# openfheorg/openfhe-development

Hardware: AMD Instinct MI355X
Metric: NTT GB/s vs HBM roofline + CKKS EvalMultKeySwitch/sec, N=2^16 L=30, 1/2/4/8 GPU (higher is better)
Workload: dtype u64; 1 GPU; batched fwd+inv negacyclic NTT, N=2^16, L=30 x 60-bit limbs, 1024 polynomials per GPU (BASELINE configs[1]); global_batch=1024, parallelism=batch-sharded x1, no data-path collective

## Files before the change

openfhe-development_amd/csrc/basis_kernels.h:

```cpp
#ifndef FHE_BASIS_KERNELS_H
#define FHE_BASIS_KERNELS_H
#include <type_traits>

#include "modarith.h"
#include "launch.h"
#include "ntt_kernels.h"
#include "elemwise_kernels.h"
#include "ntt_static.h"

namespace fhe {


struct ConvTables {
    const TwPair* hatInv;
    const uint64_t* hatMod;
    const uint64_t* srcQ;
    const uint64_t* dstQ;
    const uint64_t* dstMu;
    const uint64_t* dstRed;
    const double* srcQInv;
    const uint64_t* alphaMod;
};

struct ConvArgs {
    const uint64_t* in;
    uint64_t* out;
    ConvTables tb;
    uint32_t logN, batch;
    uint32_t nSrc, nDst;
    uint32_t inStride, inFirst, outStride, outFirst;
    uint32_t acc;
    uint32_t last;
    uint32_t nSrcAll;
    const uint64_t* inAll;
    const TwPair* allHatInv;
    const uint64_t* allSrcQ;
    const double* allQInv;
};

template <int NSRC, bool EXACT, int SUM8 = 2, bool CHUNK = false>
FHE_GLOBAL void FHE_LAUNCH_BOUNDS(kThreads) switch_basis_kernel(const ConvArgs g) {
    const uint32_t N     = 1u << g.logN;
    const uint64_t gid   = (uint64_t)FHE_BID * kThreads + FHE_TID;
    if (gid >= ((uint64_t)g.batch << g.logN))
        return;
    const uint32_t b  = (uint32_t)(gid >> g.logN);
    const uint32_t ri = (uint32_t)gid & (N - 1u);
    const uint64_t* in = g.in + (((uint64_t)b * g.inStride + g.inFirst) << g.logN) + ri;
    uint64_t* out      = g.out + (((uint64_t)b * g.outStride + g.outFirst) << g.logN) + ri;

    uint64_t xin[NSRC];
#pragma unroll
    for (int i = 0; i < NSRC; ++i) {
        const uint32_t row = (uint32_t)i < g.nSrc ? (uint32_t)i : g.nSrc - 1u;
        xin[i]             = in[(uint64_t)row << g.logN];
    }
    uint64_t y[NSRC];
    double nu = 0.5;
    const uint64_t* hp = reinterpret_cast<const uint64_t*>(g.tb.hatInv);
#pragma unroll
    for (int i = 0; i < NSRC; ++i) {
        const uint64_t w = FHE_ULOAD64(hp, 2 * i), wp = FHE_ULOAD64(hp, 2 * i + 1), qi = FHE_ULOAD64(g.tb.srcQ, i);
        const double qinv = EXACT ? FHE_ULOADF64(g.tb.srcQInv, i) : 0.0;
        y[i] = 0;
        if (i < (int)g.nSrc) {
            y[i] = mul_shoup(xin[i], w, wp, qi);
            if (EXACT)
                nu += (double)y[i] * qinv;
        }
    }
    if (CHUNK && EXACT && g.last) {
        nu = 0.5;
        const uint64_t* hpa = reinterpret_cast<const uint64_t*>(g.allHatInv);
        const uint64_t* ina = g.inAll + (((uint64_t)b * g.inStride) << g.logN) + ri;
        for (uint32_t i = 0; i < g.nSrcAll; ++i) {
            const uint64_t yi = mul_shoup(ina[(uint64_t)i << g.logN], hpa[2 * i], hpa[2 * i + 1], g.allSrcQ[i]);
            nu += (double)yi * g.allQInv[i];
        }
    }
    const uint32_t alpha = EXACT && (!CHUNK || g.last) ? (uint32_t)nu : 0u;

    for (uint32_t j = 0; j < g.nDst; ++j) {
        uint64_t h[NSRC];
#pragma unroll
        for (int i = 0; i < NSRC; ++i)
            h[i] = FHE_ULOAD64(g.tb.hatMod, (uint64_t)j * NSRC + i);
        const uint64_t p = FHE_ULOAD64(g.tb.dstQ, j);
        const uint64_t mulo = FHE_ULOAD64(g.tb.dstMu, 2 * j), muhi = FHE_ULOAD64(g.tb.dstMu, 2 * j + 1);
        if (SUM8 == 2) {
            const uint32_t k = 64u - (uint32_t)__builtin_clzll(p);
            uint64_t v       = 0;
#pragma unroll
            for (int c0 = 0; c0 < NSRC; c0 += 8) {
                if (c0 && c0 >= (int)g.nSrc)
                    break;
                sum8s s8;
                sum8s_clear(s8);
#pragma unroll
                for (int i = c0; i < c0 + 8 && i < NSRC; ++i) {
                    uint32_t y0, y1, h0, h1;
                    split30(y[i], y0, y1);
                    split30(h[i], h0, h1);
                    sum8s_add(s8, y0, y1, h0, h1);
                }
                const uint64_t rj = sum8s_reduce(s8, p, k, mulo, muhi);
                v                 = c0 ? add_mod(v, rj, p) : rj;
            }
            if (CHUNK && g.acc)
                v = add_mod(v, out[(uint64_t)j << g.logN], p);
            if (EXACT && (!CHUNK || g.last))
                v = sub_mod(v, g.tb.alphaMod[(uint64_t)alpha * g.nDst + j], p);
            out[(uint64_t)j << g.logN] = v;
            continue;
        }
        {
            static_assert(SUM8 == 1 || SUM8 == 2, "SUM8 selects one of the two column-sum forms");
            const uint32_t k = 64u - (uint32_t)__builtin_clzll(p);
            uint64_t v       = 0;
#pragma unroll
            for (int c0 = 0; c0 < NSRC; c0 += 8) {
                if (c0 && c0 >= (int)g.nSrc)
                    break;
                sum8 s8;
                sum8_clear(s8);
#pragma unroll
                for (int i = c0; i < c0 + 8 && i < NSRC; ++i)
                    sum8_add(s8, y[i], h[i]);
                const uint64_t rj = sum8_reduce(s8, p, k, mulo, muhi);
                v                 = c0 ? add_mod(v, rj, p) : rj;
            }
            if (CHUNK && g.acc)
                v = add_mod(v, out[(uint64_t)j << g.logN], p);
            if (EXACT && (!CHUNK || g.last))
                v = sub_mod(v, g.tb.alphaMod[(uint64_t)alpha * g.nDst + j], p);
            out[(uint64_t)j << g.logN] = v;
        }
    }
}

constexpr int kMaxDigits = 8;
struct KsInnerArgs {
    const uint64_t* c;
    const uint64_t* digits[kMaxDigits];
    const uint64_t* keyB;
    const uint64_t* keyA;
    uint64_t* out0;
    uint64_t* out1;
    const LimbConst* lc;
    const uint64_t* mu128;
    const uint64_t* red;
    uint32_t logN, batch, sizeQl, sizeQ, sizeP, numDigits, alpha;
    uint32_t nc[kMaxDigits];
    uint32_t j0, acc;
};
FHE_GLOBAL void FHE_LAUNCH_BOUNDS(kThreads) ks_inner_product_kernel(const KsInnerArgs g) {
    const uint32_t t          = FHE_TID;
    const uint32_t tilesPerRow = (1u << g.logN) >> kTileLog ? ((1u << g.logN) >> kTileLog) : 1u;
    const uint32_t sizeQlP    = g.sizeQl + g.sizeP;
    const uint32_t xcd = FHE_BID & 7u, slot = FHE_BID >> 3;
    const uint32_t b   = slot % g.batch;
    const uint32_t grp = (slot / g.batch) * 8u + xcd;
    const uint32_t tr = grp % tilesPerRow;
    const uint32_t i  = grp / tilesPerRow;
    if (i >= sizeQlP)
        return;
    const uint32_t idx  = i < g.sizeQl ? i : i + (g.sizeQ - g.sizeQl);
    const LimbConst lc  = g.lc[idx];
    const uint64_t mulo = g.mu128[2 * idx], muhi = g.mu128[2 * idx + 1];
    const uint64_t redc = g.red[idx];
    const uint32_t redM = (uint32_t)redc, redR = (uint32_t)(redc >> 32);
    FHE_BOUND_CHECK(redR == 255u || redR >= 3u, "key switch: the quotient estimate on a modulus below 36 bits");
    const uint32_t N    = 1u << g.logN;
    const uint32_t rEnd = ((tr + 1u) << kTileLog) < N ? ((tr + 1u) << kTileLog) : N;
    const uint64_t q = lc.q;
    for (uint32_t r = (tr << kTileLog) + t; r < rEnd; r += kThreads) {
        sum8 s0, s1;
        sum8_clear(s0);
        sum8_clear(s1);
        for (uint32_t j = 0; j < g.numDigits; ++j) {
            const uint32_t start = (g.j0 + j) * g.alpha;
            const uint32_t sz    = sizeQlP - g.nc[j];
            uint64_t d;
            if (i >= start && i < start + sz)
                d = g.c[(((uint64_t)b * g.sizeQl + i) << g.logN) + r];
            else {
                const uint32_t pos = i < start ? i : i - sz;
                d = g.digits[j][(((uint64_t)b * g.nc[j] + pos) << g.logN) + r];
            }
            if (redR != 255u)
                d -= (uint64_t)((uint32_t)(((d >> 32) * redM) >> 32) >> redR) * q;
            else {
                d = csub(d, q << 3);
                d = csub(d, q << 2);
                d = csub(d, q << 1);
            }
            d = csub(d, q);
            FHE_BOUND_CHECK(d < q, "key switch: a digit of q or more enters the 64-bit column sums");
            const uint64_t koff = (((uint64_t)(g.j0 + j) * (g.sizeQ + g.sizeP) + idx) << g.logN) + r;
            sum8_add(s0, d, g.keyB[koff]);
            sum8_add(s1, d, g.keyA[koff]);
        }
        const uint64_t ooff = (((uint64_t)b * sizeQlP + i) << g.logN) + r;
        uint64_t v0 = sum8_reduce(s0, q, lc.msb, mulo, muhi), v1 = sum8_reduce(s1, q, lc.msb, mulo, muhi);
        if (g.acc) {
            v0 = add_mod(v0, g.out0[ooff], q);
            v1 = add_mod(v1, g.out1[ooff], q);
        }
        g.out0[ooff] = v0;
        g.out1[ooff] = v1;
    }
}

constexpr int kMaxMultiKeys = 16;
struct KsInnerMultiArgs {
    const uint64_t* c;
    const uint64_t* digits[kMaxDigits];
    const uint64_t* keyB[kMaxMultiKeys];
    const uint64_t* keyA[kMaxMultiKeys];
    uint64_t* out0[kMaxMultiKeys];
    uint64_t* out1[kMaxMultiKeys];
    const uint64_t* first;
    const TwPair* firstC;
    const LimbConst* lc;
    const uint64_t* mu128;
    const uint64_t* red;
    uint32_t logN, batch, sizeQl, sizeQ, sizeP, numDigits, alpha, nKeys;
    uint32_t nc[kMaxDigits];
};
struct alignas(16) U64x2 {
    uint64_t a, b;
};
template <int CPL>
FHE_HD void ld_cpl(const uint64_t* p, uint64_t (&v)[CPL]) {
    if constexpr (CPL == 2) {
        const U64x2 w = *reinterpret_cast<const U64x2*>(p);
        v[0] = w.a, v[1] = w.b;
    }
    else
        v[0] = p[0];
}
template <int CPL>
FHE_HD void st_cpl(uint64_t* p, const uint64_t (&v)[CPL]) {
    if constexpr (CPL == 2)
        *reinterpret_cast<U64x2*>(p) = U64x2{v[0], v[1]};
    else
        p[0] = v[0];
}
template <int ND, int CPL = 1, bool PF = true>
FHE_GLOBAL void FHE_LAUNCH_BOUNDS(kThreads) ks_inner_multi_kernel(const KsInnerMultiArgs g) {
    const uint32_t t           = FHE_TID;
    const uint32_t tilesPerRow = (1u << g.logN) >> kTileLog ? ((1u << g.logN) >> kTileLog) : 1u;
    const uint32_t sizeQlP     = g.sizeQl + g.sizeP;
    const uint32_t xcd = FHE_BID & 7u, slot = FHE_BID >> 3;
    const uint32_t b   = slot % g.batch;
    const uint32_t grp = (slot / g.batch) * 8u + xcd;
    const uint32_t tr = grp % tilesPerRow;
    const uint32_t i  = grp / tilesPerRow;
    if (i >= sizeQlP)
        return;
    const uint32_t idx  = i < g.sizeQl ? i : i + (g.sizeQ - g.sizeQl);
    const LimbConst lc  = g.lc[idx];
    const uint64_t mulo = g.mu128[2 * idx], muhi = g.mu128[2 * idx + 1];
    const uint64_t redc = g.red[idx];
    const uint32_t redM = (uint32_t)redc, redR = (uint32_t)(redc >> 32);
    FHE_BOUND_CHECK(redR == 255u || redR >= 3u, "key switch: the quotient estimate on a modulus below 36 bits");
    const bool addFirst = g.first != nullptr && i < g.sizeQl;
    TwPair fc{0, 0};
    if (addFirst)
        fc = g.firstC[i];
    const uint32_t N    = 1u << g.logN;
    const uint32_t rEnd = ((tr + 1u) << kTileLog) < N ? ((tr + 1u) << kTileLog) : N;
    const uint64_t q = lc.q;
    const uint64_t ooff0 = ((uint64_t)b * sizeQlP + i) << g.logN;
    const uint64_t* src[ND];
    uint64_t koffJ[ND];
#pragma unroll
    for (int j = 0; j < ND; ++j) {
        const uint32_t jj    = (uint32_t)j < g.numDigits ? (uint32_t)j : g.numDigits - 1u;
        const uint32_t start = jj * g.alpha;
        const uint32_t sz    = sizeQlP - g.nc[jj];
        const bool own       = i >= start && i < start + sz;
        const uint32_t pos   = i < start ? i : i - sz;
        src[j] = own ? g.c + (((uint64_t)b * g.sizeQl + i) << g.logN) : g.digits[jj] + (((uint64_t)b * g.nc[jj] + pos) << g.logN);
        koffJ[j] = ((uint64_t)jj * (g.sizeQ + g.sizeP) + idx) << g.logN;
    }
    const uint64_t* firstRow = addFirst ? g.first + (((uint64_t)b * g.sizeQl + i) << g.logN) : nullptr;
    for (uint32_t r = (tr << kTileLog) + CPL * t; r < rEnd; r += CPL * kThreads) {
        uint64_t d[ND][CPL];
#pragma unroll
        for (int j = 0; j < ND; ++j)
            ld_cpl<CPL>(src[j] + r, d[j]);
        uint64_t fraw[CPL] = {};
        if (addFirst)
            ld_cpl<CPL>(firstRow + r, fraw);
        uint64_t kb[ND][CPL], ka[ND][CPL], nb[ND][CPL], na[ND][CPL];
#pragma unroll
        for (int j = 0; j < ND; ++j) {
            ld_cpl<CPL>(g.keyB[0] + koffJ[j] + r, kb[j]);
            ld_cpl<CPL>(g.keyA[0] + koffJ[j] + r, ka[j]);
        }
// ... 458 lines not shown
```

openfhe-development_amd/csrc/fhe_hip.cpp:

```cpp
#include "../../include/fhe_hip.h"

#include <algorithm>
#include <cmath>
#include <cstdio>
#include <cstdlib>
#include <map>
#include <mutex>
#include <shared_mutex>
#include <string>
#include <type_traits>
#include <vector>

#include "basis_kernels.h"
#include "bfv_kernels.h"
#include "elemwise_kernels.h"
#include "host_math.h"
#include "keygen_kernels.h"
#include "encrypt_kernels.h"
#include "decrypt_kernels.h"
#include "ntt_kernels.h"
#include "ntt_static.h"
#include "ntt_row8.h"
#include "rt.h"
#include "sampler_kernels.h"
// ... 1475 lines not shown
    a.nBlocks = kind == 0 ? (a.total + 255) / 256 : (a.total + 511) / 512;
    return kind == 0   ? blake2_launch<0>(c, a, key, counter0, st)
           : kind == 1 ? blake2_launch<1>(c, a, key, counter0, st)
                       : blake2_launch<2>(c, a, key, counter0, st);
}
extern "C" fhe_status fhe_sample_uniform_blake2(fhe_ctx* c, uint64_t* out, const uint32_t* li, uint32_t nl, uint32_t bt,
                                                const uint32_t key[16], uint64_t counter0, void* st) {
    return blake2_sample(c, out, li, nl, bt, 0, 0.0, key, counter0, st, "fhe_sample_uniform_blake2");
}
extern "C" fhe_status fhe_sample_gaussian_blake2(fhe_ctx* c, uint64_t* out, const uint32_t* li, uint32_t nl, uint32_t bt, double sigma,
                                                 const uint32_t key[16], uint64_t counter0, void* st) {
    return blake2_sample(c, out, li, nl, bt, 1, sigma, key, counter0, st, "fhe_sample_gaussian_blake2");
}
extern "C" fhe_status fhe_sample_ternary_blake2(fhe_ctx* c, uint64_t* out, const uint32_t* li, uint32_t nl, uint32_t bt,
                                                const uint32_t key[16], uint64_t counter0, void* st) {
    return blake2_sample(c, out, li, nl, bt, 2, 0.0, key, counter0, st, "fhe_sample_ternary_blake2");
}

struct fhe_conv {
    fhe_ctx* ctx;
    uint32_t nSrc, nDst;
    std::vector<uint32_t> srcIdx, dstIdx;
    ConvTables tb;
    std::vector<ConvTables> chunks;
    const TwPair* allHatInv  = nullptr;
    const uint64_t* allSrcQ  = nullptr;
    const double* allQInv    = nullptr;
    std::vector<void*> owned;
};

static uint32_t conv_nsrc_pad(uint32_t nSrc) { return nSrc <= 8 ? 8u : nSrc <= 16 ? 16u : 32u; }
static fhe_status conv_from_tables(fhe_ctx* c, const std::vector<uint64_t>& src, const std::vector<uint64_t>& dst,
                                   const uint64_t* hatInvIn, const uint64_t* hatModIn, const uint64_t* alphaIn,
                                   const double* qInvIn, fhe_conv** out) {
    const uint32_t nSrc = (uint32_t)src.size(), nDst = (uint32_t)dst.size();
    if (nSrc < 1 || nSrc > (uint32_t)kMaxLimbs || nDst < 1 || nDst > (uint32_t)kMaxLimbs)
        return fail(FHE_ERR_ARG, "basis conversion: 1..256 source and target limbs");
    fhe_conv* cv = new fhe_conv;
    cv->ctx      = c;
    cv->nSrc     = nSrc;
    cv->nDst     = nDst;
    std::vector<uint64_t> mu(2 * (size_t)nDst), alphaMod((size_t)(nSrc + 1) * nDst, 0), red(4 * (size_t)nDst);
    for (uint32_t j = 0; j < nDst; ++j) {
        host::mu128(dst[j], &mu[2 * j]);
        const uint64_t R = (uint64_t)((((unsigned __int128)1) << 64) % dst[j]);
        red[4 * j]       = dst[j];
        red[4 * j + 1]   = R;
        red[4 * j + 2]   = host::shoup(R, dst[j]);
        red[4 * j + 3]   = (uint64_t)((((unsigned __int128)1) << 64) / dst[j]);
    }
    if (alphaIn)
        for (size_t k = 0; k < alphaMod.size(); ++k)
            alphaMod[k] = alphaIn[k] % dst[k % nDst];
    ConvTables shared{};
    fhe_status s;
    if ((s = dev_copy(&cv->owned, dst.data(), dst.size(), &shared.dstQ)) ||
        (s = dev_copy(&cv->owned, mu.data(), mu.size(), &shared.dstMu)) ||
        (s = dev_copy(&cv->owned, red.data(), red.size(), &shared.dstRed)) ||
        (s = dev_copy(&cv->owned, alphaMod.data(), alphaMod.size(), &shared.alphaMod))) {
        fhe_conv_destroy(cv);
        return s;
    }
    for (uint32_t c0 = 0; c0 < nSrc; c0 += 32u) {
        const uint32_t n   = std::min(32u, nSrc - c0);
        const uint32_t pad = conv_nsrc_pad(n);
        std::vector<TwPair> hatInv(32, TwPair{0, 0});
        std::vector<uint64_t> hatMod((size_t)pad * nDst, 0), srcPad(32, 1);
        std::vector<double> qInv(32, 0.0);
        for (uint32_t i = 0; i < n; ++i) {
            const uint64_t inv = hatInvIn[c0 + i] % src[c0 + i];
            hatInv[i]          = TwPair{inv, host::shoup(inv, src[c0 + i])};
            qInv[i]            = qInvIn ? qInvIn[c0 + i] : 1.0 / static_cast<double>(src[c0 + i]);
            srcPad[i]          = src[c0 + i];
            for (uint32_t j = 0; j < nDst; ++j)
                hatMod[(size_t)j * pad + i] = hatModIn[(size_t)(c0 + i) * nDst + j] % dst[j];
        }
        ConvTables tb = shared;
        if ((s = dev_copy(&cv->owned, hatInv.data(), hatInv.size(), &tb.hatInv)) ||
            (s = dev_copy(&cv->owned, hatMod.data(), hatMod.size(), &tb.hatMod)) ||
            (s = dev_copy(&cv->owned, srcPad.data(), srcPad.size(), &tb.srcQ)) ||
            (s = dev_copy(&cv->owned, qInv.data(), qInv.size(), &tb.srcQInv))) {
            fhe_conv_destroy(cv);
            return s;
        }
        cv->chunks.push_back(tb);
    }
    cv->tb = cv->chunks[0];
    if (nSrc > 32u) {
        std::vector<TwPair> allInv(nSrc);
        std::vector<double> allQInv(nSrc);
        for (uint32_t i = 0; i < nSrc; ++i) {
            const uint64_t inv = hatInvIn[i] % src[i];
            allInv[i]          = TwPair{inv, host::shoup(inv, src[i])};
            allQInv[i]         = qInvIn ? qInvIn[i] : 1.0 / static_cast<double>(src[i]);
        }
        if ((s = dev_copy(&cv->owned, allInv.data(), allInv.size(), &cv->allHatInv)) ||
            (s = dev_copy(&cv->owned, src.data(), src.size(), &cv->allSrcQ)) ||
            (s = dev_copy(&cv->owned, allQInv.data(), allQInv.size(), &cv->allQInv))) {
            fhe_conv_destroy(cv);
            return s;
        }
    }
    *out = cv;
    return FHE_OK;
}
static fhe_status conv_build(fhe_ctx* c, const std::vector<uint64_t>& src, const std::vector<uint64_t>& dst, fhe_conv** out,
                             const uint64_t* srcScale = nullptr, const uint64_t* dstScale = nullptr) {
    const uint32_t nSrc = (uint32_t)src.size(), nDst = (uint32_t)dst.size();
    std::vector<uint64_t> hatInv(nSrc), hatMod((size_t)nSrc * nDst), alphaMod((size_t)(nSrc + 1) * nDst);
    for (uint32_t i = 0; i < nSrc; ++i) {
        const uint64_t hat = host::prod_mod(src, (int)i, src[i]);
        hatInv[i]          = host::invmod(hat, src[i]);
        if (srcScale)
            hatInv[i] = host::mulmod(hatInv[i], srcScale[i] % src[i], src[i]);
        for (uint32_t j = 0; j < nDst; ++j) {
            uint64_t v = host::prod_mod(src, (int)i, dst[j]);
            if (dstScale)
                v = host::mulmod(v, dstScale[j] % dst[j], dst[j]);
            hatMod[(size_t)i * nDst + j] = v;
        }
    }
    for (uint32_t j = 0; j < nDst; ++j) {
        const uint64_t Qmod = host::prod_mod(src, -1, dst[j]);
        for (uint32_t a = 0; a <= nSrc; ++a)
            alphaMod[(size_t)a * nDst + j] = host::mulmod(a % dst[j], Qmod, dst[j]);
    }
    return conv_from_tables(c, src, dst, hatInv.data(), hatMod.data(), alphaMod.data(), nullptr, out);
}

extern "C" fhe_status fhe_conv_create(fhe_ctx* c, const uint32_t* srcIdx, uint32_t nSrc, const uint32_t* dstIdx,
                                      uint32_t nDst, fhe_conv** out) {
    ARG_CHECK(c && srcIdx && dstIdx && out, "fhe_conv_create: null argument");
    ARG_CHECK(nSrc >= 1 && nSrc <= (uint32_t)kMaxLimbs && nDst >= 1 && nDst <= (uint32_t)kMaxLimbs, "fhe_conv_create: bad basis size");
    std::vector<uint64_t> src(nSrc), dst(nDst);
    for (uint32_t i = 0; i < nSrc; ++i) {
        ARG_CHECK(srcIdx[i] < c->L, "fhe_conv_create: source limb exceeds context size");
        src[i] = c->q[srcIdx[i]];
    }
    for (uint32_t j = 0; j < nDst; ++j) {
        ARG_CHECK(dstIdx[j] < c->L, "fhe_conv_create: target limb exceeds context size");
        dst[j] = c->q[dstIdx[j]];
    }
    RT_CHECK(rt::set_device(c->device));
    if (fhe_status s = conv_build(c, src, dst, out))
        return s;
    (*out)->srcIdx.assign(srcIdx, srcIdx + nSrc);
    (*out)->dstIdx.assign(dstIdx, dstIdx + nDst);
    return FHE_OK;
}
extern "C" fhe_status fhe_conv_create_custom(fhe_ctx* c, const uint32_t* srcIdx, uint32_t nSrc, const uint32_t* dstIdx,
                                             uint32_t nDst, const uint64_t* hatInv, const uint64_t* hatMod,
                                             const uint64_t* alphaMod, const double* qInv, fhe_conv** out) {
    ARG_CHECK(c && srcIdx && dstIdx && hatInv && hatMod && out, "fhe_conv_create_custom: null argument");
    ARG_CHECK(nSrc >= 1 && nSrc <= (uint32_t)kMaxLimbs && nDst >= 1 && nDst <= (uint32_t)kMaxLimbs, "fhe_conv_create_custom: bad basis size");
    ARG_CHECK((alphaMod == nullptr) == (qInv == nullptr), "fhe_conv_create_custom: alphaMod and qInv go together");
    std::vector<uint64_t> src(nSrc), dst(nDst);
    for (uint32_t i = 0; i < nSrc; ++i) {
        ARG_CHECK(srcIdx[i] < c->L, "fhe_conv_create_custom: source limb exceeds context size");
        src[i] = c->q[srcIdx[i]];
    }
    for (uint32_t j = 0; j < nDst; ++j) {
        ARG_CHECK(dstIdx[j] < c->L, "fhe_conv_create_custom: target limb exceeds context size");
        dst[j] = c->q[dstIdx[j]];
    }
    RT_CHECK(rt::set_device(c->device));
    if (fhe_status s = conv_from_tables(c, src, dst, hatInv, hatMod, alphaMod, qInv, out))
        return s;
    (*out)->srcIdx.assign(srcIdx, srcIdx + nSrc);
    (*out)->dstIdx.assign(dstIdx, dstIdx + nDst);
    return FHE_OK;
}
extern "C" void fhe_conv_destroy(fhe_conv* cv) {
    if (!cv)
        return;
    for (void* p : cv->owned)
        rt::dfree(p);
    delete cv;
}

template <bool EXACT>
static fhe_status conv_run(fhe_conv* cv, const uint64_t* in, uint32_t inStride, uint32_t inFirst, uint64_t* out,
                           uint32_t outStride, uint32_t outFirst, uint32_t batch, void* st) {
    ARG_CHECK(cv && in && out, "fhe_switch_basis: null argument");
    ARG_CHECK(batch >= 1 && inFirst + cv->nSrc <= inStride && outFirst + cv->nDst <= outStride,
              "fhe_switch_basis: limb window exceeds tower stride");
    RT_CHECK(rt::set_device(cv->ctx->device));
    ConvArgs g{};
    g.in = in, g.out = out, g.tb = cv->tb;
    g.logN = cv->ctx->logN, g.batch = batch, g.nSrc = cv->nSrc, g.nDst = cv->nDst;
    g.inStride = inStride, g.inFirst = inFirst, g.outStride = outStride, g.outFirst = outFirst;
    const uint64_t coeffs = (uint64_t)batch << g.logN;
    const uint32_t grid   = (uint32_t)((coeffs + kThreads - 1) / kThreads);
    static const bool split30 = env_u32("FHE_CONV_SUM8", 2) != 1u;
    if (cv->chunks.size() > 1) {
        g.nSrcAll = cv->nSrc, g.inAll = in + ((size_t)inFirst << g.logN);
        g.allHatInv = cv->allHatInv, g.allSrcQ = cv->allSrcQ, g.allQInv = cv->allQInv;
        for (size_t k = 0; k < cv->chunks.size(); ++k) {
            g.tb      = cv->chunks[k];
            g.nSrc    = std::min(32u, cv->nSrc - 32u * (uint32_t)k);
            g.inFirst = inFirst + 32u * (uint32_t)k;
            g.acc     = k > 0;
            g.last    = k + 1 == cv->chunks.size();
            const uint32_t pad = conv_nsrc_pad(g.nSrc);
            if (pad == 8)
                FHE_LAUNCH((switch_basis_kernel<8, EXACT, 2, true>), grid, st, g);
            else if (pad == 16)
                FHE_LAUNCH((switch_basis_kernel<16, EXACT, 2, true>), grid, st, g);
            else
                FHE_LAUNCH((switch_basis_kernel<32, EXACT, 2, true>), grid, st, g);
            LAUNCH_CHECK();
        }
        return FHE_OK;
    }
    const uint32_t pad = conv_nsrc_pad(cv->nSrc);
    if (pad == 8 && split30)
        FHE_LAUNCH((switch_basis_kernel<8, EXACT, 2>), grid, st, g);
    else if (pad == 8)
        FHE_LAUNCH((switch_basis_kernel<8, EXACT, 1>), grid, st, g);
    else if (pad == 16 && split30)
        FHE_LAUNCH((switch_basis_kernel<16, EXACT, 2>), grid, st, g);
    else if (pad == 16)
        FHE_LAUNCH((switch_basis_kernel<16, EXACT, 1>), grid, st, g);
    else if (split30)
        FHE_LAUNCH((switch_basis_kernel<32, EXACT, 2>), grid, st, g);
    else
        FHE_LAUNCH((switch_basis_kernel<32, EXACT, 1>), grid, st, g);
    LAUNCH_CHECK();
    return FHE_OK;
}
extern "C" fhe_status fhe_approx_switch_basis(fhe_conv* cv, const uint64_t* in, uint32_t is, uint32_t ifst,
                                              uint64_t* out, uint32_t os, uint32_t ofst, uint32_t b, void* st) {
    return conv_run<false>(cv, in, is, ifst, out, os, ofst, b, st);
}
extern "C" fhe_status fhe_switch_basis_exact(fhe_conv* cv, const uint64_t* in, uint32_t is, uint32_t ifst,
                                             uint64_t* out, uint32_t os, uint32_t ofst, uint32_t b, void* st) {
    return conv_run<true>(cv, in, is, ifst, out, os, ofst, b, st);
}

extern "C" size_t fhe_expand_crt_basis_workspace_bytes(const fhe_conv* cv, uint32_t batch) {
    return cv ? (((size_t)batch * cv->nSrc) << cv->ctx->logN) * 8 : 0;
}
static fhe_status expand_run(fhe_conv* cv, const uint64_t* x, int inEval, uint64_t* out, int resultEval, int reverseOrder,
                             uint32_t batch, void* ws, size_t wsBytes, void* st, bool exact) {
    ARG_CHECK(cv && x && out && batch >= 1, "fhe_expand_crt_basis: bad argument");
    ARG_CHECK(!cv->srcIdx.empty(), "fhe_expand_crt_basis: the plan must come from fhe_conv_create[_custom]");
    fhe_ctx* c = cv->ctx;
    RT_CHECK(rt::set_device(c->device));
    const uint32_t nQ = cv->nSrc, nP = cv->nDst, tot = nQ + nP;
    const uint32_t qFirst = reverseOrder ? nP : 0, pFirst = reverseOrder ? 0 : nQ;
    const size_t rowB = (size_t)8 << c->logN;
    const uint64_t* coef = x;
    if (inEval) {
        ARG_CHECK(ws && wsBytes >= fhe_expand_crt_basis_workspace_bytes(cv, batch), "fhe_expand_crt_basis: workspace too small");
        if (fhe_status s = ntt_run(c, true, x, (uint64_t*)ws, cv->srcIdx.data(), nQ, batch, st))
            return s;
        coef = (const uint64_t*)ws;
    }
    if (fhe_status s = exact ? conv_run<true>(cv, coef, nQ, 0, out, tot, pFirst, batch, st)
                             : conv_run<false>(cv, coef, nQ, 0, out, tot, pFirst, batch, st))
        return s;
    const uint64_t* qsrc = (resultEval && inEval) ? x : coef;
    uint64_t* qdst       = out + ((size_t)qFirst << c->logN);
    RT_CHECK(rt::d2d_2d(qdst, tot * rowB, qsrc, nQ * rowB, nQ * rowB, batch, (rt::stream_t)st));
    if (resultEval) {
        NttOpts rows;
        rows.src.stride = rows.dst.stride = tot;
        rows.src.first = rows.dst.first = qFirst;
        if (!inEval)
            if (fhe_status s = ntt_run(c, false, out, out, cv->srcIdx.data(), nQ, batch, st, rows))
                return s;
        rows.src.first = rows.dst.first = pFirst;
        return ntt_run(c, false, out, out, cv->dstIdx.data(), nP, batch, st, rows);
    }
    return FHE_OK;
}
extern "C" fhe_status fhe_expand_crt_basis(fhe_conv* cv, const uint64_t* x, int inEval, uint64_t* out, int resultEval,
                                           int reverseOrder, uint32_t batch, void* ws, size_t wsBytes, void* st) {
    return expand_run(cv, x, inEval, out, resultEval, reverseOrder, batch, ws, wsBytes, st, true);
}
// ... 2784 lines not shown
    behz_moduli(h, q, bsk);
    fhe_status s;
    if ((s = behz_pairs(h, mtildeQHatInvModq, q.data(), h->numQ, &h->tb.mtQHatInv)) ||
        (s = behz_matrix(h, QHatModbsk, h->numQ, h->numBsk, bsk.data(), &h->tb.QHatModbsk)) ||
        (s = behz_pairs(h, QModbsk, bsk.data(), h->numBsk, &h->tb.QModbsk)) ||
        (s = behz_pairs(h, mtildeInvModbsk, bsk.data(), h->numBsk, &h->tb.mtInvModbsk)))
        return s;
    std::vector<uint64_t> mt(h->tb.W, 0);
    std::copy(QHatModmtilde, QHatModmtilde + h->numQ, mt.begin());
    uint64_t* d = nullptr;
    if ((s = dev_copy(&h->owned, mt.data(), mt.size(), &d)))
        return s;
    h->tb.QHatModmt    = d;
    h->tb.negQInvModmt = negQInvModmtilde;
    return FHE_OK;
}
extern "C" fhe_status fhe_behz_override_floorq(fhe_behz* h, const uint64_t* tQHatInvModq, const uint64_t* QHatModbsk,
                                               const uint64_t* qInvModbsk, const uint64_t* tQInvModbsk) {
    ARG_CHECK(h && tQHatInvModq && QHatModbsk && qInvModbsk && tQInvModbsk, "fhe_behz_override_floorq: null argument");
    RT_CHECK(rt::set_device(h->ctx->device));
    std::vector<uint64_t> q, bsk;
    behz_moduli(h, q, bsk);
    fhe_status s;
    if ((s = behz_pairs(h, tQHatInvModq, q.data(), h->numQ, &h->tb.tQHatInv)) ||
        (s = behz_matrix(h, QHatModbsk, h->numQ, h->numBsk, bsk.data(), &h->tb.QHatModbsk)) ||
        (s = behz_matrix(h, qInvModbsk, h->numQ, h->numBsk, bsk.data(), &h->tb.qInvModbsk)) ||
        (s = behz_pairs(h, tQInvModbsk, bsk.data(), h->numBsk, &h->tb.tQInvModbsk)))
        return s;
    return FHE_OK;
}
extern "C" fhe_status fhe_behz_override_conv_sk(fhe_behz* h, const uint64_t* BHatInvModb, const uint64_t* BHatModmsk, uint64_t BInvModmsk,
                                                const uint64_t* BHatModq, const uint64_t* BModq) {
    ARG_CHECK(h && BHatInvModb && BHatModmsk && BHatModq && BModq, "fhe_behz_override_conv_sk: null argument");
    RT_CHECK(rt::set_device(h->ctx->device));
    std::vector<uint64_t> q, bsk;
    behz_moduli(h, q, bsk);
    const uint32_t numB = h->numQ;
    const uint64_t msk  = bsk[numB];
    fhe_status s;
    if ((s = behz_pairs(h, BHatInvModb, bsk.data(), numB, &h->tb.BHatInv)) ||
        (s = behz_matrix(h, BHatModq, numB, h->numQ, q.data(), &h->tb.BHatModq)) || (s = behz_pairs(h, BModq, q.data(), h->numQ, &h->tb.BModq)))
        return s;
    std::vector<uint64_t> bm(h->tb.W, 0);
    for (uint32_t i = 0; i < numB; ++i)
        bm[i] = BHatModmsk[i] % msk;
    uint64_t* d = nullptr;
    if ((s = dev_copy(&h->owned, bm.data(), bm.size(), &d)))
        return s;
    h->tb.BHatModmsk = d;
    h->tb.BInvModmsk = TwPair{BInvModmsk % msk, host::shoup(BInvModmsk % msk, msk)};
    return FHE_OK;
}
static bool behz_split30() {
    static const bool on = env_u32("FHE_CONV_SUM8", 2) != 1u;
    return on;
}
static uint32_t coeff_grid(const fhe_ctx* c, uint32_t batch) {
    return (uint32_t)((((uint64_t)batch << c->logN) + kThreads - 1) / kThreads);
}
extern "C" size_t fhe_behz_workspace_bytes(const fhe_behz* h, uint32_t batch) {
    return h ? ((size_t)batch * h->numQ << h->ctx->logN) * 8 : 0;
}
extern "C" fhe_status fhe_behz_q_to_bsk(fhe_behz* h, uint64_t* x, int evalFormat, uint32_t batch, void* ws, size_t wsBytes,
                                        void* st) {
    ARG_CHECK(h && x && batch >= 1, "fhe_behz_q_to_bsk: bad argument");
    fhe_ctx* c = h->ctx;
    RT_CHECK(rt::set_device(c->device));
    const uint32_t tot = h->numQ + h->numBsk;
    BehzArgs g;
    g.tb = h->tb, g.logN = c->logN, g.batch = batch;
    g.outBsk = TowerView{x, tot, h->numQ};
    g.inBsk = g.outBsk, g.outQ = TowerView{x, tot, 0};
    if (evalFormat) {
        ARG_CHECK(ws && wsBytes >= fhe_behz_workspace_bytes(h, batch), "fhe_behz_q_to_bsk: workspace too small");
        uint64_t* coef = (uint64_t*)ws;
        NttOpts rows;
        rows.src.stride = tot, rows.src.first = 0;
        if (fhe_status s = ntt_run(c, true, x, coef, h->qIdx.data(), h->numQ, batch, st, rows))
            return s;
        g.inQ = TowerView{coef, h->numQ, 0};
        if (h->tb.W > (uint32_t)kMaxBfvLimbs)
            FHE_LAUNCH(behz_q_to_bsk_wide_kernel, coeff_grid(c, batch), st, g);
        else if (behz_split30())
            FHE_LAUNCH((behz_q_to_bsk_kernel<true>), coeff_grid(c, batch), st, g);
        else
            FHE_LAUNCH((behz_q_to_bsk_kernel<false>), coeff_grid(c, batch), st, g);
        LAUNCH_CHECK();
        rows.dst.stride = tot, rows.src.first = rows.dst.first = h->numQ;
        return ntt_run(c, false, x, x, h->bskIdx.data(), h->numBsk, batch, st, rows);
    }
    g.inQ = TowerView{x, tot, 0};
    if (h->tb.W > (uint32_t)kMaxBfvLimbs)
        FHE_LAUNCH(behz_q_to_bsk_wide_kernel, coeff_grid(c, batch), st, g);
    else if (behz_split30())
        FHE_LAUNCH((behz_q_to_bsk_kernel<true>), coeff_grid(c, batch), st, g);
    else
        FHE_LAUNCH((behz_q_to_bsk_kernel<false>), coeff_grid(c, batch), st, g);
    LAUNCH_CHECK();
    return fhe_ntt_fwd(c, x, h->allIdx.data(), tot, batch, st);
}
extern "C" fhe_status fhe_behz_floorq(fhe_behz* h, uint64_t* x, uint32_t batch, void* st) {
    ARG_CHECK(h && x && batch >= 1, "fhe_behz_floorq: bad argument");
    RT_CHECK(rt::set_device(h->ctx->device));
    const uint32_t tot = h->numQ + h->numBsk;
    BehzArgs g;
    g.tb = h->tb, g.logN = h->ctx->logN, g.batch = batch;
    g.inQ = g.outQ = TowerView{x, tot, 0};
// ... 1127 lines not shown
```

openfhe-development_amd/csrc/modarith.h:

```cpp
#ifndef FHE_MODARITH_H
#define FHE_MODARITH_H
#include <stdint.h>

#if defined(__HIPCC__) || defined(__HIP_DEVICE_COMPILE__)
#include <hip/hip_runtime.h>
#define FHE_HD __host__ __device__ __forceinline__
#else
#define FHE_HD inline
#endif

namespace fhe {

FHE_HD uint64_t mulhi64(uint64_t a, uint64_t b) {
#if defined(__HIP_DEVICE_COMPILE__)
    return __umul64hi(a, b);
#else
    return (uint64_t)(((unsigned __int128)a * b) >> 64);
#endif
}

FHE_HD uint64_t csub(uint64_t x, uint64_t m) {
    return x >= m ? x - m : x;
}

// ... 108 lines not shown
    mac192_add(m, a, b);
}
#endif
struct u128w;
FHE_HD void mac192_fold(const mac192& m, uint64_t& lo, uint64_t& hi) {
    const uint64_t c1lo = m.c1 << 32, c1hi = (m.c1 >> 32) + ((uint64_t)m.k1 << 32);
    lo = m.c0 + c1lo;
    hi = m.c2 + c1hi + (uint64_t)m.k0 + (lo < c1lo);
}

struct sum8 {
    uint64_t c0, c1, c2;
    uint32_t k0;
};
FHE_HD void sum8_clear(sum8& s) {
    s.c0 = s.c1 = s.c2 = 0;
    s.k0 = 0;
}
FHE_HD void sum8_add(sum8& s, uint64_t x, uint64_t y) {
    const uint32_t xl = (uint32_t)x, xh = (uint32_t)(x >> 32), yl = (uint32_t)y, yh = (uint32_t)(y >> 32);
    const uint64_t lo = (uint64_t)xl * yl + s.c0;
    s.k0 += lo < s.c0;
    s.c0 = lo;
    s.c1 += (uint64_t)xl * yh;
    s.c1 += (uint64_t)xh * yl;
    s.c2 += (uint64_t)xh * yh;
}
FHE_HD uint64_t sum8_reduce(const sum8& s, uint64_t q, uint32_t k, uint64_t mu_lo, uint64_t mu_hi) {
    const uint64_t m = s.c1 << 32, lo = s.c0 + m;
    const uint64_t hi = s.c2 + (s.c1 >> 32) + s.k0 + (lo < m);
    const uint32_t sh = 65u - k;
    const uint64_t mu = (mu_lo >> sh) | (mu_hi << (64u - sh));
    const uint64_t sv = (lo >> (k - 1u)) | (hi << sh);
    uint64_t r        = lo - mulhi64(sv, mu) * q;
    r -= r >= q ? q : 0;
    r -= r >= q ? q : 0;
    return r;
}

struct sum8s {
    uint64_t c0, c1, c2;
};
FHE_HD void sum8s_clear(sum8s& s) { s.c0 = s.c1 = s.c2 = 0; }
FHE_HD void split30(uint64_t x, uint32_t& x0, uint32_t& x1) {
    x0 = (uint32_t)x & 0x3fffffffu;
    x1 = (uint32_t)(x >> 30);
}
FHE_HD void sum8s_add(sum8s& s, uint32_t x0, uint32_t x1, uint32_t y0, uint32_t y1) {
    s.c0 += (uint64_t)x0 * y0;
    s.c1 += (uint64_t)x0 * y1;
    s.c1 += (uint64_t)x1 * y0;
    s.c2 += (uint64_t)x1 * y1;
}
FHE_HD uint64_t sum8s_reduce(const sum8s& s, uint64_t q, uint32_t k, uint64_t mu_lo, uint64_t mu_hi) {
    const uint64_t t1 = s.c1 << 30, l1 = s.c0 + t1, t2 = s.c2 << 60, lo = l1 + t2;
    const uint64_t hi = (s.c1 >> 34) + (s.c2 >> 4) + (l1 < t1) + (lo < t2);
    const uint32_t sh = 65u - k;
    const uint64_t mu = (mu_lo >> sh) | (mu_hi << (64u - sh));
    const uint64_t sv = (lo >> (k - 1u)) | (hi << sh);
    uint64_t r        = lo - mulhi64(sv, mu) * q;
    r -= r >= q ? q : 0;
    r -= r >= q ? q : 0;
    return r;
}

FHE_HD uint64_t barrett128(u128w a, uint64_t q, uint64_t mu_lo, uint64_t mu_hi) {
    uint64_t left_hi = mulhi64(a.lo, mu_lo);
    uint64_t mid_lo  = a.lo * mu_hi;
    uint64_t mid_hi  = mulhi64(a.lo, mu_hi);
    uint64_t tmp1    = mid_lo + left_hi;
    uint64_t tmp2    = mid_hi + (tmp1 < mid_lo);
    uint64_t m2_lo   = a.hi * mu_lo;
    uint64_t m2_hi   = mulhi64(a.hi, mu_lo);
    uint64_t carry   = (uint64_t)(m2_lo + tmp1) < m2_lo;
    uint64_t quot    = a.hi * mu_hi + tmp2 + m2_hi + carry;
    uint64_t r       = a.lo - quot * q;
    return csub(csub(r, q), q);
}

FHE_HD uint64_t mul_mod(uint64_t a, uint64_t b, uint64_t q, uint64_t mu_lo, uint64_t mu_hi) {
    return barrett128(mul128(a, b), q, mu_lo, mu_hi);
}

FHE_HD uint64_t mul_mod_barrett(uint64_t a, uint64_t b, uint64_t q, uint64_t mu, int msb) {
    uint64_t lo = a * b, hi = mulhi64(a, b);
    int n       = msb - 2;
    uint64_t t  = (lo >> n) | (hi << (64 - n));
    uint64_t plo = t * mu, phi = mulhi64(t, mu);
    int sh       = n + 7;
    uint64_t est = sh < 64 ? ((plo >> sh) | (phi << (64 - sh))) : (phi >> (sh - 64));
    uint64_t r   = lo - est * q;
    return csub(r, q);
}

}
#endif
```

Measured before the change: 2401 GB/s.

## Use Montgomery REDC and two-coefficient lanes in basis conversion kernel

Basis conversion gets a third column-sum form. The hat-mod table is pre-scaled by 2^64 mod p so each column sum can be reduced with a Montgomery REDC instead of a 128-bit Barrett reduction. The multiply-accumulates use inline v_mad_u64_u32 with scalar-register operands, and when nSrc<=8 and pointers are 16-byte aligned each lane handles two adjacent coefficients with 128-bit loads and stores. This cuts ALU work and memory instruction count in key-switch basis conversion, at the cost of extra tables, higher register pressure, and hand-written inline asm that bypasses the compiler.

```diff
diff --git a/openfhe-development_amd/csrc/basis_kernels.h b/openfhe-development_amd/csrc/basis_kernels.h
--- a/openfhe-development_amd/csrc/basis_kernels.h
+++ b/openfhe-development_amd/csrc/basis_kernels.h
@@ -14,6 +14,8 @@
 struct ConvTables {
     const TwPair* hatInv;
     const uint64_t* hatMod;
+    const uint64_t* hatModM;
+    const uint64_t* dstNqInv;
     const uint64_t* srcQ;
     const uint64_t* dstQ;
     const uint64_t* dstMu;
@@ -38,10 +40,32 @@
     const double* allQInv;
 };
 
-template <int NSRC, bool EXACT, int SUM8 = 2, bool CHUNK = false>
+struct alignas(16) U64x2 {
+    uint64_t a, b;
+};
+template <int CPL>
+FHE_HD void ld_cpl(const uint64_t* p, uint64_t (&v)[CPL]) {
+    if constexpr (CPL == 2) {
+        const U64x2 w = *reinterpret_cast<const U64x2*>(p);
+        v[0] = w.a, v[1] = w.b;
+    }
+    else
+        v[0] = p[0];
+}
+template <int CPL>
+FHE_HD void st_cpl(uint64_t* p, const uint64_t (&v)[CPL]) {
+    if constexpr (CPL == 2)
+        *reinterpret_cast<U64x2*>(p) = U64x2{v[0], v[1]};
+    else
+        p[0] = v[0];
+}
+
+template <int NSRC, bool EXACT, int SUM8 = 2, bool CHUNK = false, int CPL = 1>
 FHE_GLOBAL void FHE_LAUNCH_BOUNDS(kThreads) switch_basis_kernel(const ConvArgs g) {
+    static_assert(SUM8 >= 1 && SUM8 <= 3, "SUM8 selects one of the three column-sum forms");
+    static_assert(CPL == 1 || CPL == 2, "one or two coefficients per lane");
     const uint32_t N     = 1u << g.logN;
-    const uint64_t gid   = (uint64_t)FHE_BID * kThreads + FHE_TID;
+    const uint64_t gid   = ((uint64_t)FHE_BID * kThreads + FHE_TID) * CPL;
     if (gid >= ((uint64_t)g.batch << g.logN))
         return;
     const uint32_t b  = (uint32_t)(gid >> g.logN);
@@ -49,92 +73,122 @@
     const uint64_t* in = g.in + (((uint64_t)b * g.inStride + g.inFirst) << g.logN) + ri;
     uint64_t* out      = g.out + (((uint64_t)b * g.outStride + g.outFirst) << g.logN) + ri;
 
-    uint64_t xin[NSRC];
+    uint64_t xin[NSRC][CPL];
 #pragma unroll
     for (int i = 0; i < NSRC; ++i) {
         const uint32_t row = (uint32_t)i < g.nSrc ? (uint32_t)i : g.nSrc - 1u;
-        xin[i]             = in[(uint64_t)row << g.logN];
-    }
-    uint64_t y[NSRC];
-    double nu = 0.5;
+        ld_cpl<CPL>(in + ((uint64_t)row << g.logN), xin[i]);
+    }
+    uint64_t y[NSRC][CPL];
+    double nu[CPL];
+#pragma unroll
+    for (int c = 0; c < CPL; ++c)
+        nu[c] = 0.5;
     const uint64_t* hp = reinterpret_cast<const uint64_t*>(g.tb.hatInv);
 #pragma unroll
     for (int i = 0; i < NSRC; ++i) {
         const uint64_t w = FHE_ULOAD64(hp, 2 * i), wp = FHE_ULOAD64(hp, 2 * i + 1), qi = FHE_ULOAD64(g.tb.srcQ, i);
         const double qinv = EXACT ? FHE_ULOADF64(g.tb.srcQInv, i) : 0.0;
-        y[i] = 0;
+#pragma unroll
+        for (int c = 0; c < CPL; ++c)
+            y[i][c] = 0;
         if (i < (int)g.nSrc) {
-            y[i] = mul_shoup(xin[i], w, wp, qi);
-            if (EXACT)
-                nu += (double)y[i] * qinv;
+#pragma unroll
+            for (int c = 0; c < CPL; ++c) {
+                y[i][c] = mul_shoup(xin[i][c], w, wp, qi);
+                if (EXACT)
+                    nu[c] += (double)y[i][c] * qinv;
+            }
         }
     }
     if (CHUNK && EXACT && g.last) {
-        nu = 0.5;
         const uint64_t* hpa = reinterpret_cast<const uint64_t*>(g.allHatInv);
         const uint64_t* ina = g.inAll + (((uint64_t)b * g.inStride) << g.logN) + ri;
+#pragma unroll
+        for (int c = 0; c < CPL; ++c)
+            nu[c] = 0.5;
         for (uint32_t i = 0; i < g.nSrcAll; ++i) {
-            const uint64_t yi = mul_shoup(ina[(uint64_t)i << g.logN], hpa[2 * i], hpa[2 * i + 1], g.allSrcQ[i]);
-            nu += (double)yi * g.allQInv[i];
-        }
-    }
-    const uint32_t alpha = EXACT && (!CHUNK || g.last) ? (uint32_t)nu : 0u;
-
+            uint64_t xa[CPL];
+            ld_cpl<CPL>(ina + ((uint64_t)i << g.logN), xa);
+#pragma unroll
+            for (int c = 0; c < CPL; ++c) {
+                const uint64_t yi = mul_shoup(xa[c], hpa[2 * i], hpa[2 * i + 1], g.allSrcQ[i]);
+                nu[c] += (double)yi * g.allQInv[i];
+            }
+        }
+    }
+    uint32_t alpha[CPL];
+#pragma unroll
+    for (int c = 0; c < CPL; ++c)
+        alpha[c] = EXACT && (!CHUNK || g.last) ? (uint32_t)nu[c] : 0u;
+
+    const uint64_t* hatMod = SUM8 == 3 ? g.tb.hatModM : g.tb.hatMod;
     for (uint32_t j = 0; j < g.nDst; ++j) {
         uint64_t h[NSRC];
 #pragma unroll
         for (int i = 0; i < NSRC; ++i)
-            h[i] = FHE_ULOAD64(g.tb.hatMod, (uint64_t)j * NSRC + i);
+            h[i] = FHE_ULOAD64(hatMod, (uint64_t)j * NSRC + i);
         const uint64_t p = FHE_ULOAD64(g.tb.dstQ, j);
-        const uint64_t mulo = FHE_ULOAD64(g.tb.dstMu, 2 * j), muhi = FHE_ULOAD64(g.tb.dstMu, 2 * j + 1);
-        if (SUM8 == 2) {
-            const uint32_t k = 64u - (uint32_t)__builtin_clzll(p);
-            uint64_t v       = 0;
-#pragma unroll
-            for (int c0 = 0; c0 < NSRC; c0 += 8) {
-                if (c0 && c0 >= (int)g.nSrc)
-                    break;
-                sum8s s8;
-                sum8s_clear(s8);
+        const uint64_t nqinv = SUM8 == 3 ? FHE_ULOAD64(g.tb.dstNqInv, j) : 0;
+        const uint64_t mulo = SUM8 != 3 ? FHE_ULOAD64(g.tb.dstMu, 2 * j) : 0, muhi = SUM8 != 3 ? FHE_ULOAD64(g.tb.dstMu, 2 * j + 1) : 0;
+        const uint32_t k = SUM8 != 3 ? 64u - (uint32_t)__builtin_clzll(p) : 0u;
+        uint64_t v[CPL];
+#pragma unroll
+        for (int c = 0; c < CPL; ++c)
+            v[c] = 0;
+#pragma unroll
+        for (int c0 = 0; c0 < NSRC; c0 += 8) {
+            if (c0 && c0 >= (int)g.nSrc)
+                break;
+            uint64_t rj[CPL];
+            if constexpr (SUM8 == 1) {
+#pragma unroll
+                for (int c = 0; c < CPL; ++c) {
+                    sum8 s8;
+                    sum8_clear(s8);
+#pragma unroll
+                    for (int i = c0; i < c0 + 8 && i < NSRC; ++i)
+                        sum8_add(s8, y[i][c], h[i]);
+                    rj[c] = sum8_reduce(s8, p, k, mulo, muhi);
+                }
+            }
+            else {
+                sum8s s8[CPL] = {};
 #pragma unroll
                 for (int i = c0; i < c0 + 8 && i < NSRC; ++i) {
-                    uint32_t y0, y1, h0, h1;
-                    split30(y[i], y0, y1);
+                    uint32_t h0, h1;
                     split30(h[i], h0, h1);
-                    sum8s_add(s8, y0, y1, h0, h1);
-                }
-                const uint64_t rj = sum8s_reduce(s8, p, k, mulo, muhi);
-                v                 = c0 ? add_mod(v, rj, p) : rj;
-            }
-            if (CHUNK && g.acc)
-                v = add_mod(v, out[(uint64_t)j << g.logN], p);
-            if (EXACT && (!CHUNK || g.last))
-                v = sub_mod(v, g.tb.alphaMod[(uint64_t)alpha * g.nDst + j], p);
-            out[(uint64_t)j << g.logN] = v;
-            continue;
-        }
-        {
-            static_assert(SUM8 == 1 || SUM8 == 2, "SUM8 selects one of the two column-sum forms");
-            const uint32_t k = 64u - (uint32_t)__builtin_clzll(p);
-            uint64_t v       = 0;
-#pragma unroll
-            for (int c0 = 0; c0 < NSRC; c0 += 8) {
-                if (c0 && c0 >= (int)g.nSrc)
-                    break;
-                sum8 s8;
-                sum8_clear(s8);
-#pragma unroll
-                for (int i = c0; i < c0 + 8 && i < NSRC; ++i)
-                    sum8_add(s8, y[i], h[i]);
-                const uint64_t rj = sum8_reduce(s8, p, k, mulo, muhi);
-                v                 = c0 ? add_mod(v, rj, p) : rj;
-            }
-            if (CHUNK && g.acc)
-                v = add_mod(v, out[(uint64_t)j << g.logN], p);
-            if (EXACT && (!CHUNK || g.last))
-                v = sub_mod(v, g.tb.alphaMod[(uint64_t)alpha * g.nDst + j], p);
-            out[(uint64_t)j << g.logN] = v;
-        }
+#pragma unroll
+                    for (int c = 0; c < CPL; ++c) {
+                        uint32_t y0, y1;
+                        split30(y[i][c], y0, y1);
+                        if (i == c0)
+                            sum8s_add_uniform<true>(s8[c], y0, y1, h0, h1);
+                        else
+                            sum8s_add_uniform<false>(s8[c], y0, y1, h0, h1);
+                    }
+                }
+#pragma unroll
+                for (int c = 0; c < CPL; ++c)
+                    rj[c] = SUM8 == 3 ? sum8s_redc(s8[c], p, nqinv) : sum8s_reduce(s8[c], p, k, mulo, muhi);
+            }
+#pragma unroll
+            for (int c = 0; c < CPL; ++c)
+                v[c] = c0 ? add_mod(v[c], rj[c], p) : rj[c];
+        }
+        if (CHUNK && g.acc) {
+            uint64_t o[CPL];
+            ld_cpl<CPL>(out + ((uint64_t)j << g.logN), o);
+#pragma unroll
+            for (int c = 0; c < CPL; ++c)
+                v[c] = add_mod(v[c], o[c], p);
+        }
+        if (EXACT && (!CHUNK || g.last)) {
+#pragma unroll
+            for (int c = 0; c < CPL; ++c)
+                v[c] = sub_mod(v[c], g.tb.alphaMod[(uint64_t)alpha[c] * g.nDst + j], p);
+        }
+        st_cpl<CPL>(out + ((uint64_t)j << g.logN), v);
     }
 }
 
@@ -227,25 +281,6 @@
     uint32_t logN, batch, sizeQl, sizeQ, sizeP, numDigits, alpha, nKeys;
     uint32_t nc[kMaxDigits];
 };
-struct alignas(16) U64x2 {
-    uint64_t a, b;
-};
-template <int CPL>
-FHE_HD void ld_cpl(const uint64_t* p, uint64_t (&v)[CPL]) {
-    if constexpr (CPL == 2) {
-        const U64x2 w = *reinterpret_cast<const U64x2*>(p);
-        v[0] = w.a, v[1] = w.b;
-    }
-    else
-        v[0] = p[0];
-}
-template <int CPL>
-FHE_HD void st_cpl(uint64_t* p, const uint64_t (&v)[CPL]) {
-    if constexpr (CPL == 2)
-        *reinterpret_cast<U64x2*>(p) = U64x2{v[0], v[1]};
-    else
-        p[0] = v[0];
-}
 template <int ND, int CPL = 1, bool PF = true>
 FHE_GLOBAL void FHE_LAUNCH_BOUNDS(kThreads) ks_inner_multi_kernel(const KsInnerMultiArgs g) {
     const uint32_t t           = FHE_TID;
diff --git a/openfhe-development_amd/csrc/fhe_hip.cpp b/openfhe-development_amd/csrc/fhe_hip.cpp
--- a/openfhe-development_amd/csrc/fhe_hip.cpp
+++ b/openfhe-development_amd/csrc/fhe_hip.cpp
@@ -1551,8 +1551,21 @@
     if (alphaIn)
         for (size_t k = 0; k < alphaMod.size(); ++k)
             alphaMod[k] = alphaIn[k] % dst[k % nDst];
+    bool allOdd = true;
+    std::vector<uint64_t> nqinv(nDst);
+    for (uint32_t j = 0; j < nDst; ++j) {
+        allOdd = allOdd && (dst[j] & 1u);
+        uint64_t inv = dst[j];
+        for (int it = 0; it < 5; ++it)
+            inv *= 2 - dst[j] * inv;
+        nqinv[j] = 0 - inv;
+    }
     ConvTables shared{};
     fhe_status s;
+    if (allOdd && (s = dev_copy(&cv->owned, nqinv.data(), nqinv.size(), &shared.dstNqInv))) {
+        fhe_conv_destroy(cv);
+        return s;
+    }
     if ((s = dev_copy(&cv->owned, dst.data(), dst.size(), &shared.dstQ)) ||
         (s = dev_copy(&cv->owned, mu.data(), mu.size(), &shared.dstMu)) ||
         (s = dev_copy(&cv->owned, red.data(), red.size(), &shared.dstRed)) ||
@@ -1564,17 +1577,24 @@
         const uint32_t n   = std::min(32u, nSrc - c0);
         const uint32_t pad = conv_nsrc_pad(n);
         std::vector<TwPair> hatInv(32, TwPair{0, 0});
-        std::vector<uint64_t> hatMod((size_t)pad * nDst, 0), srcPad(32, 1);
+        std::vector<uint64_t> hatMod((size_t)pad * nDst, 0), hatModM((size_t)pad * nDst, 0), srcPad(32, 1);
         std::vector<double> qInv(32, 0.0);
         for (uint32_t i = 0; i < n; ++i) {
             const uint64_t inv = hatInvIn[c0 + i] % src[c0 + i];
             hatInv[i]          = TwPair{inv, host::shoup(inv, src[c0 + i])};
             qInv[i]            = qInvIn ? qInvIn[c0 + i] : 1.0 / static_cast<double>(src[c0 + i]);
             srcPad[i]          = src[c0 + i];
-            for (uint32_t j = 0; j < nDst; ++j)
-                hatMod[(size_t)j * pad + i] = hatModIn[(size_t)(c0 + i) * nDst + j] % dst[j];
+            for (uint32_t j = 0; j < nDst; ++j) {
+                const uint64_t h             = hatModIn[(size_t)(c0 + i) * nDst + j] % dst[j];
+                hatMod[(size_t)j * pad + i]  = h;
+                hatModM[(size_t)j * pad + i] = (uint64_t)((((unsigned __int128)h) << 64) % dst[j]);
+            }
         }
         ConvTables tb = shared;
+        if (allOdd && (s = dev_copy(&cv->owned, hatModM.data(), hatModM.size(), &tb.hatModM))) {
+            fhe_conv_destroy(cv);
+            return s;
+        }
         if ((s = dev_copy(&cv->owned, hatInv.data(), hatInv.size(), &tb.hatInv)) ||
             (s = dev_copy(&cv->owned, hatMod.data(), hatMod.size(), &tb.hatMod)) ||
             (s = dev_copy(&cv->owned, srcPad.data(), srcPad.size(), &tb.srcQ)) ||
@@ -1677,6 +1697,29 @@
     delete cv;
 }
 
+template <bool EXACT, int SUM8, bool CHUNK, int CPL>
+static void conv_launch(const ConvArgs& g, uint32_t grid, void* st) {
+#define FHE_CONV_LAUNCH(NS)                                                                                                   \
+    do {                                                                                                                      \
+        if (CPL == 2)                                                                                                         \
+            FHE_LAUNCH_AS("CPL2", (switch_basis_kernel<NS, EXACT, SUM8, CHUNK, CPL>), grid, fhe::kThreads, false, st, g);     \
+        else                                                                                                                  \
+            FHE_LAUNCH((switch_basis_kernel<NS, EXACT, SUM8, CHUNK, CPL>), grid, st, g);                                      \
+    } while (0)
+    if constexpr (CPL == 2) {
+        FHE_CONV_LAUNCH(8);
+    }
+    else {
+        const uint32_t pad = conv_nsrc_pad(g.nSrc);
+        if (pad == 8)
+            FHE_CONV_LAUNCH(8);
+        else if (pad == 16)
+            FHE_CONV_LAUNCH(16);
+        else
+            FHE_CONV_LAUNCH(32);
+    }
+#undef FHE_CONV_LAUNCH
+}
 template <bool EXACT>
 static fhe_status conv_run(fhe_conv* cv, const uint64_t* in, uint32_t inStride, uint32_t inFirst, uint64_t* out,
                            uint32_t outStride, uint32_t outFirst, uint32_t batch, void* st) {
@@ -1689,8 +1732,11 @@
     g.logN = cv->ctx->logN, g.batch = batch, g.nSrc = cv->nSrc, g.nDst = cv->nDst;
     g.inStride = inStride, g.inFirst = inFirst, g.outStride = outStride, g.outFirst = outFirst;
     const uint64_t coeffs = (uint64_t)batch << g.logN;
-    const uint32_t grid   = (uint32_t)((coeffs + kThreads - 1) / kThreads);
-    static const bool split30 = env_u32("FHE_CONV_SUM8", 2) != 1u;
+    static const uint32_t formEnv = env_u32("FHE_CONV_SUM8", 3);
+    static const uint32_t cplEnv  = env_u32("FHE_CONV_CPL", 2);
+    const uint32_t form = formEnv == 1u ? 1u : formEnv == 2u || !cv->tb.hatModM ? 2u : 3u;
+    const bool wide     = form == 3u && cplEnv != 1u && cv->nSrc <= 8u && cv->ctx->N >= 2 && (((uintptr_t)in | (uintptr_t)out) & 15u) == 0;
+    const uint32_t grid = (uint32_t)((coeffs / (wide ? 2u : 1u) + kThreads - 1) / kThreads);
     if (cv->chunks.size() > 1) {
         g.nSrcAll = cv->nSrc, g.inAll = in + ((size_t)inFirst << g.logN);
         g.allHatInv = cv->allHatInv, g.allSrcQ = cv->allSrcQ, g.allQInv = cv->allQInv;
@@ -1700,30 +1746,22 @@
             g.inFirst = inFirst + 32u * (uint32_t)k;
             g.acc     = k > 0;
             g.last    = k + 1 == cv->chunks.size();
-            const uint32_t pad = conv_nsrc_pad(g.nSrc);
-            if (pad == 8)
-                FHE_LAUNCH((switch_basis_kernel<8, EXACT, 2, true>), grid, st, g);
-            else if (pad == 16)
-                FHE_LAUNCH((switch_basis_kernel<16, EXACT, 2, true>), grid, st, g);
+            if (form == 3u)
+                conv_launch<EXACT, 3, true, 1>(g, grid, st);
             else
-                FHE_LAUNCH((switch_basis_kernel<32, EXACT, 2, true>), grid, st, g);
+                conv_launch<EXACT, 2, true, 1>(g, grid, st);
             LAUNCH_CHECK();
         }
         return FHE_OK;
     }
-    const uint32_t pad = conv_nsrc_pad(cv->nSrc);
-    if (pad == 8 && split30)
-        FHE_LAUNCH((switch_basis_kernel<8, EXACT, 2>), grid, st, g);
-    else if (pad == 8)
-        FHE_LAUNCH((switch_basis_kernel<8, EXACT, 1>), grid, st, g);
-    else if (pad == 16 && split30)
-        FHE_LAUNCH((switch_basis_kernel<16, EXACT, 2>), grid, st, g);
-    else if (pad == 16)
-        FHE_LAUNCH((switch_basis_kernel<16, EXACT, 1>), grid, st, g);
-    else if (split30)
-        FHE_LAUNCH((switch_basis_kernel<32, EXACT, 2>), grid, st, g);
+    if (wide)
+        conv_launch<EXACT, 3, false, 2>(g, grid, st);
+    else if (form == 3u)
+        conv_launch<EXACT, 3, false, 1>(g, grid, st);
+    else if (form == 2u)
+        conv_launch<EXACT, 2, false, 1>(g, grid, st);
     else
-        FHE_LAUNCH((switch_basis_kernel<32, EXACT, 1>), grid, st, g);
+        conv_launch<EXACT, 1, false, 1>(g, grid, st);
     LAUNCH_CHECK();
     return FHE_OK;
 }
@@ -4614,7 +4652,7 @@
     return FHE_OK;
 }
 static bool behz_split30() {
-    static const bool on = env_u32("FHE_CONV_SUM8", 2) != 1u;
+    static const bool on = env_u32("FHE_CONV_SUM8", 3) != 1u;
     return on;
 }
 static uint32_t coeff_grid(const fhe_ctx* c, uint32_t batch) {
diff --git a/openfhe-development_amd/csrc/modarith.h b/openfhe-development_amd/csrc/modarith.h
--- a/openfhe-development_amd/csrc/modarith.h
+++ b/openfhe-development_amd/csrc/modarith.h
@@ -184,6 +184,35 @@
     s.c1 += (uint64_t)x1 * y0;
     s.c2 += (uint64_t)x1 * y1;
 }
+#if defined(__HIP_DEVICE_COMPILE__) && !defined(FHE_NO_MAD_ASM)
+__device__ __forceinline__ uint64_t mad64_uniform(uint32_t a, uint32_t u, uint64_t c) {
+    uint64_t d;
+    asm("v_mad_u64_u32 %0, vcc, %1, %2, %3" : "=v"(d) : "v"(a), "s"(u), "v"(c) : "vcc");
+    return d;
+}
+__device__ __forceinline__ uint64_t mul32x32_uniform(uint32_t a, uint32_t u) {
+    uint64_t d;
+    asm("v_mad_u64_u32 %0, vcc, %1, %2, 0" : "=v"(d) : "v"(a), "s"(u) : "vcc");
+    return d;
+}
+#else
+FHE_HD uint64_t mad64_uniform(uint32_t a, uint32_t u, uint64_t c) { return (uint64_t)a * u + c; }
+FHE_HD uint64_t mul32x32_uniform(uint32_t a, uint32_t u) { return (uint64_t)a * u; }
+#endif
+template <bool FIRST>
+FHE_HD void sum8s_add_uniform(sum8s& s, uint32_t x0, uint32_t x1, uint32_t u0, uint32_t u1) {
+    if (FIRST) {
+        s.c0 = mul32x32_uniform(x0, u0);
+        s.c1 = mul32x32_uniform(x0, u1);
+        s.c2 = mul32x32_uniform(x1, u1);
+    }
+    else {
+        s.c0 = mad64_uniform(x0, u0, s.c0);
+        s.c1 = mad64_uniform(x0, u1, s.c1);
+        s.c2 = mad64_uniform(x1, u1, s.c2);
+    }
+    s.c1 = mad64_uniform(x1, u0, s.c1);
+}
 FHE_HD uint64_t sum8s_reduce(const sum8s& s, uint64_t q, uint32_t k, uint64_t mu_lo, uint64_t mu_hi) {
     const uint64_t t1 = s.c1 << 30, l1 = s.c0 + t1, t2 = s.c2 << 60, lo = l1 + t2;
     const uint64_t hi = (s.c1 >> 34) + (s.c2 >> 4) + (l1 < t1) + (lo < t2);
@@ -194,6 +223,12 @@
     r -= r >= q ? q : 0;
     r -= r >= q ? q : 0;
     return r;
+}
+FHE_HD uint64_t sum8s_redc(const sum8s& s, uint64_t q, uint64_t nqinv) {
+    const uint64_t t1 = s.c1 << 30, l1 = s.c0 + t1, t2 = s.c2 << 60, lo = l1 + t2;
+    const uint64_t hi = (s.c1 >> 34) + (s.c2 >> 4) + (l1 < t1) + (lo < t2);
+    const uint64_t m  = lo * nqinv;
+    return csub(hi + mulhi64(m, q) + (lo != 0), q);
 }
 
 FHE_HD uint64_t barrett128(u128w a, uint64_t q, uint64_t mu_lo, uint64_t mu_hi) {
```

Result: no change. 2403 GB/s, median of 2 (+0.1%).
